# zihuixue/DynMM

Hardware: AMD Instinct MI355X
Metric: images/sec fwd+bwd, 480x640 RGB-D, batch 32/GPU (higher is better)
Workload: dtype f32; 1 GPU; configs[2]: zero-grad + fwd + weighted 4-scale CE + FLOP loss + bwd + fused SGD-Nesterov update, --dynamic --global-gate soft DiffSoftmax gates tau=1; per_gpu_batch=32, global_batch=32, height=480, width=640, parallelism=dp1, launch=eager, streams=4, optimizer_in_step=fused SGD-Nesterov

## Files before the change

### dynmm_amd/lib.py

```python
import ctypes as C
import os
import subprocess

_HERE = os.path.dirname(os.path.abspath(__file__))
LIB_PATH = os.path.join(_HERE, 'libdynmm_hip.so')
CSRC = os.path.join(_HERE, 'csrc')

ACT_NONE, ACT_RELU, ACT_TANH, ACT_SWISH, ACT_HSWISH = 0, 1, 2, 3, 4
SMOOTH_ACTS = (ACT_SWISH, ACT_HSWISH)
DYNMM_OK, DYNMM_EINVAL, DYNMM_EUNSUPPORTED, DYNMM_EWORKSPACE = 0, -1, -2, -3
ACT = {None: 0, 'none': 0, 'relu': 1, 'tanh': 2, 'swish': 3, 'silu': 3, 'hswish': 4}
LOSS_BCE_LOGITS, LOSS_L1 = 0, 1

c_f = C.c_void_p
c_i = C.c_int
c_fl = C.c_float
c_sz = C.c_size_t
c_ll = C.c_longlong


class ConvGeom(C.Structure):
    _fields_ = [(n, C.c_int) for n in ('N', 'Ci', 'H', 'W', 'Co', 'Ho', 'Wo',
                                       'KH', 'KW', 'SH', 'SW', 'PH', 'PW', 'c_split')]


class Dropout(C.Structure):
    _fields_ = [('mask', C.c_void_p), ('step', C.c_void_p), ('seed', C.c_ulonglong), ('offset', C.c_ulonglong),
                ('p', C.c_float)]


_GP = C.POINTER(ConvGeom)
_DP = C.POINTER(Dropout)
_PP = C.POINTER(C.c_void_p)
_IP = C.POINTER(C.c_int)

SIGNATURES = {
    'dynmm_abi_version': (c_i, []),
    'dynmm_build_info': (C.c_char_p, []),
    'dynmm_debug_set_igemm_v5': (c_i, [c_i]),
    'dynmm_conv2d_uses_operand_ring': (c_i, [_GP, c_i]),
    'dynmm_packed_weight_floats': (c_sz, [c_i, c_i, c_i, c_i, c_i]),
    'dynmm_pack_weight': (c_i, [c_f, c_f, c_f, c_i, c_i, c_i, c_i, c_f]),
    'dynmm_pack_weight_multi': (c_i, [c_f, c_f, c_f, c_i, c_i, c_f]),
    'dynmm_pack_weight_multi_blocks': (c_i, [c_i] * 5),
    'dynmm_conv2d_fwd': (c_i, [c_f, c_f, c_f, c_f, c_f, c_f, c_f, _GP, c_i, c_f]),
    'dynmm_conv2d_stem_fwd_stats_supported': (c_i, [_GP]),
    'dynmm_conv2d_stem_fwd_stats': (c_i, [c_f, c_f, c_f, c_f, c_f, _GP, c_f]),
    'dynmm_conv2d_dgrad': (c_i, [c_f, c_f, c_f, c_f, c_f, c_f, _GP, c_f]),
    'dynmm_conv2d_wino_supported': (c_i, [_GP, c_i]),
    'dynmm_wino_packed_floats': (c_sz, [c_i, c_i, c_i, c_i]),
    'dynmm_wino_pack': (c_i, [c_f, c_f, c_f, c_i, c_i, c_i, c_i, c_i, c_f]),
    'dynmm_wino_pack_multi_blocks': (c_i, [c_i] * 4),
    'dynmm_wino_pack_multi': (c_i, [c_f, c_f, c_f, c_i, c_i, c_f]),
    'dynmm_conv2d_wino_fwd': (c_i, [c_f, c_f, c_f, c_f, c_f, _GP, c_i, c_f]),
    'dynmm_conv2d_wino_dgrad_bnred_supported': (c_i, [_GP]),
    'dynmm_conv2d_wino_dgrad_bnred_slots': (c_i, [_GP]),
    'dynmm_conv2d_wino_dgrad_bnred': (c_i, [c_f] * 9 + [_GP, c_f]),
    'dynmm_conv2d_wino_dgrad_bnred2': (c_i, [c_f] * 9 + [_GP, c_f]),
    'dynmm_conv2d_wino_fwd_stats_supported': (c_i, [_GP]),
    'dynmm_conv2d_wino_fwd_stats_slots': (c_i, [_GP]),
    'dynmm_conv2d_wino_fwd_stats': (c_i, [c_f, c_f, c_f, c_f, c_f, c_i, _GP, c_f]),
    'dynmm_conv2d_wino_dgrad': (c_i, [c_f, c_f, c_f, c_f, c_f, _GP, c_f]),
    'dynmm_conv2d_wino2d_supported': (c_i, [_GP, c_i]),
    'dynmm_wino2d_packed_floats': (c_sz, [c_i, c_i]),
    'dynmm_wino2d_pack': (c_i, [c_f, c_f, c_f, c_i, c_i, c_i, c_f]),
    'dynmm_wino2d_pack_multi_blocks': (c_i, [c_i, c_i, c_i]),
    'dynmm_wino2d_pack_multi': (c_i, [c_f, c_f, c_f, c_i, c_i, c_f]),
    'dynmm_conv2d_wino2d_stats_slots': (c_i, [_GP]),
    'dynmm_conv2d_wino2d_fwd': (c_i, [c_f, c_f, c_f, c_f, c_f, c_f, c_i, _GP, c_i, c_f]),
    'dynmm_conv2d_wino2d_dgrad': (c_i, [c_f, c_f, c_f, c_f, c_f, _GP, c_f]),
    'dynmm_conv2d_wino43_supported': (c_i, [_GP]),
    'dynmm_wino43_packed_floats': (c_sz, [c_i, c_i, c_i, c_i]),
    'dynmm_wino43_pack': (c_i, [c_f, c_f, c_i, c_i, c_i, c_i, c_f]),
    'dynmm_wino43_pack_multi_blocks': (c_i, [c_i] * 4),
    'dynmm_wino43_pack_multi': (c_i, [c_f, c_f, c_f, c_i, c_i, c_f]),
    'dynmm_conv2d_wino43_dgrad': (c_i, [c_f, c_f, c_f, c_f, c_f, _GP, c_f]),
    'dynmm_conv2d_wgrad_workspace_bytes': (c_sz, [_GP]),
    'dynmm_conv2d_wgrad': (c_i, [c_f, c_f, c_f, c_f, c_f, c_f, c_sz, _GP, c_f]),
    'dynmm_conv2d_wgrad_groupable': (c_i, [_GP]),
    'dynmm_conv2d_wgrad_variant': (c_i, [_GP]),
    'dynmm_conv2d_wgrad_group_workspace_bytes': (c_sz, [_GP, c_i]),
    'dynmm_conv2d_wgrad_group': (c_i, [c_i, c_f, c_f, c_f, c_f, c_f, c_sz, _GP, c_f]),
    'dynmm_act_bwd_bias_workspace_bytes': (c_sz, [c_i, c_i]),
    'dynmm_act_bwd_bias': (c_i, [c_f, c_f, c_f, c_f, c_f, c_i, c_i, c_i, c_i, c_f]),
    'dynmm_act_pre_fwd': (c_i, [c_f, c_f, c_i, c_i, c_i, c_i, c_f]),
    'dynmm_act_pre_bwd': (c_i, [c_f, c_f, c_f, c_f, c_f, c_i, c_i, c_i, c_i, c_f]),
    'dynmm_bn_stats': (c_i, [c_f, c_f, c_i, c_i, c_i, c_i, c_f]),
    'dynmm_bn_stats_f64': (c_i, [c_f, c_f, c_i, c_i, c_i, c_i, c_f]),
    'dynmm_bn_relu_bits_words': (c_sz, [c_i, c_i, c_i]),
    'dynmm_bn_apply': (c_i, [c_f] * 11 + [c_i, c_i, c_i, c_fl, c_fl, c_i, c_i, c_f, c_f]),
    'dynmm_bn_bwd_reduce': (c_i, [c_f] * 8 + [c_i, c_i, c_i, c_i, c_i, c_f, c_f]),
    'dynmm_bn_bwd_apply': (c_i, [c_f] * 12 + [c_i, c_i, c_i, c_i, c_i, c_f, c_f]),
    'dynmm_bn_bwd_reduce_pre': (c_i, [c_f] * 8 + [c_i, c_i, c_i, c_i, c_i, c_f]),
    'dynmm_bn_bwd_apply_pre': (c_i, [c_f] * 12 + [c_i, c_i, c_i, c_i, c_i, c_f]),
    'dynmm_bn_fold': (c_i, [c_f] * 7 + [c_i, c_fl, c_f]),
    'dynmm_maxpool3x3s2_fwd': (c_i, [c_f, c_f, c_f] + [c_i] * 6 + [c_f]),
    'dynmm_maxpool3x3s2_bwd': (c_i, [c_f, c_f, c_f] + [c_i] * 6 + [c_f]),
    'dynmm_adaptive_avgpool_fwd': (c_i, [c_f, c_f] + [c_i] * 5 + [c_f]),
    'dynmm_adaptive_avgpool_bwd': (c_i, [c_f, c_f] + [c_i] * 5 + [c_f]),
    'dynmm_nearest_into_fwd': (c_i, [c_f, c_f] + [c_i] * 8 + [c_f]),
    'dynmm_nearest_into_bwd': (c_i, [c_f, c_f] + [c_i] * 8 + [c_f]),
# ... 176 lines not shown
```

### dynmm_amd/nn/blocks.py

```python
import torch
import torch.nn as nn

from .. import ops

ACTIVATIONS = {'relu': 'relu', 'swish': 'swish', 'silu': 'swish', 'hswish': 'hswish'}


def normalize_activation(activation):
    key = activation.lower() if isinstance(activation, str) else activation
    if key not in ACTIVATIONS:
        raise NotImplementedError('Only relu, swish and hswish as activation function are supported so far. '
                                  'Got {}'.format(activation))
    return ACTIVATIONS[key]


def conv_bn_act(x, conv, bn, act=None, residual=None, x2=None, mask_input=False, conv_link=None, res_link=None, bwd_link=None):
    if not bn.training and not torch.is_grad_enabled():
        return ops.conv2d_fused_eval(x, conv.weight, conv.bias, bn, act, residual,
                                     conv.stride, conv.padding, x2)
    y = ops.conv2d(x, conv.weight, conv.bias, conv.stride, conv.padding, None, x2, mask_input=mask_input, link=conv_link,
                   bn_stats=bn.training)
    return ops.batch_norm_act(y, bn, act, residual, link=res_link, bwd_link=bwd_link)


class ConvBNAct(nn.Sequential):

    def __init__(self, cin, cout, kernel_size, activation='relu'):
        super().__init__()
        self.activation = normalize_activation(activation)
        self.add_module('conv', nn.Conv2d(cin, cout, kernel_size, padding=kernel_size // 2, bias=False))
        self.add_module('bn', nn.BatchNorm2d(cout))

    def forward(self, x):
        return conv_bn_act(x, self.conv, self.bn, self.activation)


class NonBottleneck1D(nn.Module):
    expansion = 1

    def __init__(self, inplanes, planes, stride=1, downsample=None, activation='relu'):
        super().__init__()
        self.activation = normalize_activation(activation)
        self.conv3x1_1 = nn.Conv2d(inplanes, planes, (3, 1), stride=(stride, 1), padding=(1, 0))
        self.conv1x3_1 = nn.Conv2d(planes, planes, (1, 3), stride=(1, stride), padding=(0, 1))
        self.bn1 = nn.BatchNorm2d(planes, eps=1e-3)
        self.conv3x1_2 = nn.Conv2d(planes, planes, (3, 1), padding=(1, 0))
        self.conv1x3_2 = nn.Conv2d(planes, planes, (1, 3), padding=(0, 1))
        self.bn2 = nn.BatchNorm2d(planes, eps=1e-3)
        self.downsample = downsample

    def forward(self, x, chain=False):
        act = self.activation
        grad = torch.is_grad_enabled() and x.requires_grad
        fuse_bwd = grad and act == 'relu'
        link = ops.GradLink() if (grad and self.downsample is None) else None
        in_link = getattr(x, '_bn_out_link', None) if (chain and link is not None and fuse_bwd) else None
        xd = x
        if self.downsample is not None:
            x, xd = ops.fan_out(x, 2)
        c = self.conv3x1_1
        y = ops.conv2d(x, c.weight, c.bias, c.stride, c.padding, act, defer_mask=fuse_bwd, link=link, bn_link=in_link)
        bnl = ops.BNLink() if (fuse_bwd and self.bn1.training) else None
        y = conv_bn_act(y, self.conv1x3_1, self.bn1, act, mask_input=fuse_bwd, bwd_link=bnl)
        c = self.conv3x1_2
        y = ops.conv2d(y, c.weight, c.bias, c.stride, c.padding, act, defer_mask=fuse_bwd, bn_link=bnl)
        idt = x if self.downsample is None else conv_bn_act(xd, self.downsample[0], self.downsample[1])
        out_link = ops.BNLink() if (fuse_bwd and self.bn2.training) else None
        out = conv_bn_act(y, self.conv1x3_2, self.bn2, act, residual=idt, mask_input=fuse_bwd, res_link=link, bwd_link=out_link)
        if out_link is not None and out_link.bits is not None:
            out._bn_out_link = out_link
        return out


class BasicBlock(nn.Module):
    expansion = 1

    def __init__(self, inplanes, planes, stride=1, downsample=None, activation='relu'):
        super().__init__()
        self.activation = normalize_activation(activation)
        self.conv1 = nn.Conv2d(inplanes, planes, 3, stride=stride, padding=1, bias=False)
        self.bn1 = nn.BatchNorm2d(planes)
        self.conv2 = nn.Conv2d(planes, planes, 3, padding=1, bias=False)
        self.bn2 = nn.BatchNorm2d(planes)
        self.downsample = downsample

    def forward(self, x, chain=False):
        fuse_bwd = torch.is_grad_enabled() and x.requires_grad
        link = ops.GradLink() if (fuse_bwd and self.downsample is None) else None
        xd = x
        if self.downsample is not None:
            x, xd = ops.fan_out(x, 2)
        y = conv_bn_act(x, self.conv1, self.bn1, self.activation, conv_link=link)
        idt = x if self.downsample is None else conv_bn_act(xd, self.downsample[0], self.downsample[1])
        return conv_bn_act(y, self.conv2, self.bn2, self.activation, residual=idt, res_link=link)


class Bottleneck(nn.Module):
    expansion = 4

    def __init__(self, inplanes, planes, stride=1, downsample=None, activation='relu'):
        super().__init__()
        self.activation = normalize_activation(activation)
        self.conv1 = nn.Conv2d(inplanes, planes, 1, bias=False)
        self.bn1 = nn.BatchNorm2d(planes)
        self.conv2 = nn.Conv2d(planes, planes, 3, stride=stride, padding=1, bias=False)
        self.bn2 = nn.BatchNorm2d(planes)
        self.conv3 = nn.Conv2d(planes, planes * self.expansion, 1, bias=False)
        self.bn3 = nn.BatchNorm2d(planes * self.expansion)
        self.downsample = downsample

    def forward(self, x, chain=False):
        fuse_bwd = torch.is_grad_enabled() and x.requires_grad
        link = ops.GradLink() if (fuse_bwd and self.downsample is None) else None
        xd = x
        if self.downsample is not None:
            x, xd = ops.fan_out(x, 2)
        y = conv_bn_act(x, self.conv1, self.bn1, self.activation, conv_link=link)
        y = conv_bn_act(y, self.conv2, self.bn2, self.activation)
        idt = x if self.downsample is None else conv_bn_act(xd, self.downsample[0], self.downsample[1])
        return conv_bn_act(y, self.conv3, self.bn3, self.activation, residual=idt, res_link=link)


def chain_ok(prev, blk):
    import torch.nn.modules.module as M
    if prev._forward_hooks or blk._forward_pre_hooks:
        return False
    if M._global_forward_hooks or M._global_forward_pre_hooks:
        return False
    return True


BLOCKS = {'NonBottleneck1D': NonBottleneck1D, 'BasicBlock': BasicBlock, 'Bottleneck': Bottleneck}
LAYERS = {'resnet18': (2, 2, 2, 2), 'resnet34': (3, 4, 6, 3), 'resnet50': (3, 4, 6, 3)}


class ResNetEncoder(nn.Module):

    def __init__(self, name, block, input_channels=3, activation='relu'):
        super().__init__()
        self.activation = normalize_activation(activation)
        if name not in LAYERS:
            raise NotImplementedError(f'Only {sorted(LAYERS)} encoders are implemented on the HIP path. Got {name}')
        if block not in BLOCKS and name != 'resnet50':
            raise NotImplementedError(f'Block {block} is not implemented')
        if name == 'resnet50':
            block = 'Bottleneck'
        blk = BLOCKS[block]
        ex = blk.expansion
        self.conv1 = nn.Conv2d(input_channels, 64, 7, stride=2, padding=3, bias=False)
        self.bn1 = nn.BatchNorm2d(64)
        inplanes = 64
        for j, (planes, n) in enumerate(zip((64, 128, 256, 512), LAYERS[name]), start=1):
            stride = 1 if j == 1 else 2
            down = None
            if stride != 1 or inplanes != planes * ex:
                down = nn.Sequential(nn.Conv2d(inplanes, planes * ex, 1, stride=stride, bias=False),
                                     nn.BatchNorm2d(planes * ex))
            stage = [blk(inplanes, planes, stride, down, activation=self.activation)] + \
                [blk(planes * ex, planes, activation=self.activation) for _ in range(n - 1)]
            setattr(self, f'layer{j}', nn.Sequential(*stage))
            inplanes = planes * ex
        self.down_2_channels_out = 64
        self.down_4_channels_out, self.down_8_channels_out = 64 * ex, 128 * ex
        self.down_16_channels_out, self.down_32_channels_out = 256 * ex, 512 * ex
        for m in self.modules():
            if isinstance(m, nn.Conv2d):
                nn.init.kaiming_normal_(m.weight, mode='fan_out', nonlinearity='relu')
            elif isinstance(m, nn.BatchNorm2d):
                nn.init.constant_(m.weight, 1)
                nn.init.constant_(m.bias, 0)

    def forward_first_conv(self, x):
# ... 20 lines not shown
```

### dynmm_amd/ops.py

```python
import collections
import contextlib
import ctypes as C

import torch
from torch.autograd import Function

from . import lib as L

ACT = L.ACT


def _lib():
    return L.load()


def _stream():
    if not torch.cuda.is_available():
        raise L.DynmmHipError('no HIP device is available: the DynMM hot path runs only on its HIP kernels '
                              '(there is no CPU / eager-PyTorch fallback)')
    h = torch.cuda.current_stream().cuda_stream
    _CENSUS.add(h)
    return h


# ... 478 lines not shown

@contextlib.contextmanager
def capture_scope():
    import gc
    was = gc.isenabled()
    gc.collect()
    gc.disable()
    try:
        yield
    finally:
        if was:
            gc.enable()


ACT_TRACE = None

PROFILE = None


def _tile(co, m=1 << 30):
    if co > 64:
        return '128x32' if -(-co // 128) * -(-m // 64) < 3 * 256 else '128x64'
    return '64x128' if co > 32 else '32x256'




def _timed(kind, g, call, nprob=1, extra=0, route='direct'):
    if PROFILE is None:
        return call()
    co = g.Ci if kind == 'dgrad' else g.Co
    gemm_ci = g.Co if kind == 'dgrad' else g.Ci
    rk = ((gemm_ci + 15) & ~15) if (gemm_ci >= 8 and gemm_ci % 16) else gemm_ci
    generic = ''
    if kind != 'wgrad':
        if rk % 16 != 0 or (g.c_split < g.Ci and g.c_split % 16 != 0):
            generic = ',generic'
        elif rk != gemm_ci:
            generic = ',padded'
    m = g.N * (g.H * g.W if kind == 'dgrad' else g.Ho * g.Wo)
    name = f'conv_wgrad<co{_tile(co).split("x")[0]}>' if kind == 'wgrad' else f'conv_igemm_{kind}<{_tile(co, m)}{generic}>'
    if kind == 'wgrad':
        variant = _lib().dynmm_conv2d_wgrad_variant(C.byref(g))
        if variant == 6 and (g.SH == 2 or g.SW == 2):
            name = f'conv_wgrad_s2<co{128 if g.Co % 128 == 0 else 64},{g.KH}x{g.KW}>'
        elif variant == 6:
            name = f'conv_wgrad_v6<co{128 if g.Co % 128 == 0 else 64},{g.KH}x{g.KW}>'
        elif variant == 4:
            name = 'conv_wgrad_v4<co128>'
        elif variant == 8:
            name = 'conv_co8_wgrad<direct,valu>'
    if kind != 'wgrad' and not generic and _lib().dynmm_conv2d_uses_operand_ring(C.byref(g), int(kind == 'dgrad')):
        name = f'conv_igemm_v5_{kind}<{"128x64" if co % 128 == 0 else "64x128"},kw{g.KW}>'
    if route == 'wino2d':
        name = f'conv_wino2d_{kind}<co{128 if co % 128 == 0 else 64},3x3>'
    elif route != 'direct':
        name = f'conv_wino{"43" if route == "wino43" else ""}_{kind}<co{128 if co % 128 == 0 else 64},{g.KH}x{g.KW}{"s2" if g.SH * g.SW > 1 else ""}>'
    if kind == 'fwd':
        k5, k7 = (g.KH, g.KW, g.SH, g.SW, g.PH, g.PW) == (5, 5, 2, 2, 0, 0), (g.KH, g.KW, g.SH, g.SW, g.PH, g.PW) == (7, 7, 2, 2, 3, 3)
        if k5 and 5 <= g.Co <= 8 and g.Ci % 4 == 0 and g.Ci >= 16 and (g.c_split == g.Ci or g.c_split % (g.Ci // 4) == 0):
            name = 'conv_co8_fwd<direct,valu>'
        elif k7 and g.Ci in (1, 3) and g.Co == 64 and g.c_split == g.Ci:
            name = f'conv_stem_fwd<ci{g.Ci},mfma>'
    flops = 2.0 * g.N * g.Ho * g.Wo * g.KH * g.KW * g.Ci * g.Co * nprob
    e0, e1 = torch.cuda.Event(enable_timing=True), torch.cuda.Event(enable_timing=True)
    e0.record()
    r = call()
    e1.record()
    PROFILE.append((name, flops, e0, e1, (g.N, g.Ci, g.H, g.W, g.Co, g.KH, g.KW, g.SH, g.SW, nprob), (kind, int(extra))))
    return r


def _up4(v):
    return (v + 3) & ~3


def _pair(v):
    return (v, v) if isinstance(v, int) else tuple(v)


def _same_shape(a, b, what):
    if b is not None and tuple(a.shape) != tuple(b.shape):
        raise L.DynmmHipError(f'{what}: shape mismatch {tuple(a.shape)} vs {tuple(b.shape)}')


def _geom(x, x2, weight, stride, padding):
    if x.dim() != 4 or weight.dim() != 4:
        raise L.DynmmHipError('conv2d expects NCHW input and OIHW weight')
    if x2 is not None and (x2.shape[0] != x.shape[0] or tuple(x2.shape[2:]) != tuple(x.shape[2:])):
        raise L.DynmmHipError(f'conv2d: second input {tuple(x2.shape)} does not match {tuple(x.shape)}')
    N, C0, H, W = x.shape
    Ci = C0 + (x2.shape[1] if x2 is not None else 0)
    Co, Ciw, KH, KW = weight.shape
    if Ciw != Ci:
        raise L.DynmmHipError(f'conv2d: weight expects {Ciw} input channels, got {Ci}')
    SH, SW = stride
    PH, PW = padding
    Ho = (H + 2 * PH - KH) // SH + 1
    Wo = (W + 2 * PW - KW) // SW + 1
    if N <= 0 or Ho <= 0 or Wo <= 0:
        raise L.DynmmHipError(f'conv2d: empty output for input {tuple(x.shape)}, kernel {(KH, KW)}, stride {stride}, '
                              f'padding {padding}')
    g = L.ConvGeom(N, Ci, H, W, Co, Ho, Wo, KH, KW, SH, SW, PH, PW, C0)
    return g


class GradLink:
    __slots__ = ('dres',)

    def __init__(self):
        self.dres = None


class BNLink:
    __slots__ = ('x', 'mean', 'invstd', 'gamma', 'beta', 'sums', 'bits', 'premasked')

    def __init__(self):
        self.x = self.mean = self.invstd = self.gamma = self.beta = self.sums = self.bits = None
        self.premasked = False


BN_BWD_FUSE = True
BN_RELU_BITS = True


_PackedEntry = collections.namedtuple('_PackedEntry', 'weight Co Ci KH KW kinds')


class PackedWeights:

    def __init__(self):
        self.reg = {}
        self.slots = {}
        self.arena = None
        self.launches = []
        self.valid = False
        self.dirty = False

    def register(self, weight, g, kinds):
        if not isinstance(weight, torch.nn.Parameter):
            return
        e = self.reg.get(id(weight))
        if e is None:
            e = self.reg[id(weight)] = _PackedEntry(weight, g.Co, g.Ci, g.KH, g.KW, set())
        if not e.kinds.issuperset(kinds):
            e.kinds.update(kinds)
            self.dirty = True

    def lookup(self, weight, kinds):
        ops = self.slots.get(id(weight)) if self.valid else None
        if ops is not None:
            for kind in kinds:
                if kind not in ops:
                    return None
        return ops

    def _layout(self):
        lib = _lib()
        ents = list(self.reg.values())
        dev = ents[0].weight.device
        base = min(e.weight.data_ptr() for e in ents)
        off = 0
        rows = {name: [] for name in ('pack_weight',) + tuple(f.name + '_pack' for f in _PACK_FAMILIES)}
        blk = dict.fromkeys(rows, 0)
# ... 42 lines not shown


def _planes(t):
    if t.dim() >= 2:
        return t.shape[0], t.shape[1], max(t.numel() // max(t.shape[0] * t.shape[1], 1), 1)
    return 1, max(t.numel(), 1), 1


class _Activation(Function):

    @staticmethod
    def forward(ctx, z, act):
        z = _chk(z, 'z')
        a = torch.empty_like(z)
        if z.numel():
            N, Cc, HW = _planes(z)
            L.check(_lib().dynmm_act_pre_fwd(_p(z), _p(a), N, Cc, HW, act, _stream()), 'act_pre_fwd')
        ctx.act = act
        ctx.save_for_backward(z)
        return a

    @staticmethod
    def backward(ctx, g):
        z, = ctx.saved_tensors
        g = _chk(g, 'grad')
        dz = torch.empty_like(z)
        if z.numel():
            N, Cc, HW = _planes(z)
            L.check(_lib().dynmm_act_pre_bwd(_p(g), _p(z), _p(dz), None, None, N, Cc, HW, ctx.act, _stream()), 'act_pre_bwd')
        return dz, None


def is_smooth(act):
    return ACT[act] in L.SMOOTH_ACTS


def activation(x, act):
    code = ACT[act]
    if code == L.ACT_NONE:
        return x
    if not (torch.is_grad_enabled() and x.requires_grad):
        x = _chk(x, 'x')
        a = torch.empty_like(x)
        if x.numel():
            N, Cc, HW = _planes(x)
            L.check(_lib().dynmm_act_pre_fwd(_p(x), _p(a), N, Cc, HW, code, _stream()), 'act_pre_fwd')
        return a
    return _Activation.apply(x, code)


class _Conv2d(Function):
    @staticmethod
    def forward(ctx, x, x2, weight, bias, stride, padding, act, mask_input, defer_mask, link, w_owner=None, stats=None,
                bn_link=None):
        lib = _lib()
        st = _stream()
        x, x2, weight, bias = _chk(x, 'x'), _chk(x2, 'x2'), _chk(weight, 'weight'), _chk(bias, 'bias')
        g = _geom(x, x2, weight, stride, padding)
        need_dx = ctx.needs_input_grad[0] or (x2 is not None and ctx.needs_input_grad[1])
        y = torch.empty((g.N, g.Co, g.Ho, g.Wo), device=x.device, dtype=torch.float32)
        fwd = _fwd_route(g, x2, x.data_ptr() % 16 == 0)
        dgrad = _dgrad_route(g, x2) if need_dx else None
        kinds = (_FWD_KIND[fwd], _DGRAD_KIND[dgrad]) if need_dx else (_FWD_KIND[fwd],)
        wkey = w_owner if w_owner is not None else weight
        prepack = _STEP.prepack if _STEP is not None else None
        packed = prepack.lookup(wkey, kinds) if prepack is not None else None
        if packed is None:
            packed = _pack_operands(weight, g, kinds)
            if prepack is not None:
                prepack.register(wkey, g, kinds)
        wf = packed[kinds[0]]
        if fwd == 'wino2d':
            sums, ns = None, 0
            if stats is not None and act == L.ACT_NONE and g.Co % 64 == 0:
                ns = lib.dynmm_conv2d_wino2d_stats_slots(C.byref(g))
                stats['sums'] = sums = _zeroed_sums(2 * g.Co * ns, x.device)
            L.check(_timed('fwd', g, lambda: lib.dynmm_conv2d_wino2d_fwd(_p(x), _p(wf), _p(bias), None, _p(y), _p(sums), ns,
                                                                         C.byref(g), act, st), route=fwd), 'conv2d_wino2d_fwd')
        elif (fwd == 'wino' and stats is not None and act == L.ACT_NONE and g.KW == 3 and
                lib.dynmm_conv2d_wino_fwd_stats_supported(C.byref(g))):
            ns = lib.dynmm_conv2d_wino_fwd_stats_slots(C.byref(g))
            sums = _zeroed_sums(2 * g.Co * ns, x.device)
            L.check(_timed('fwd', g, lambda: lib.dynmm_conv2d_wino_fwd_stats(_p(x), _p(wf), _p(bias), _p(y), _p(sums), ns,
                                                                             C.byref(g), st), route=fwd), 'conv2d_wino_fwd_stats')
            stats['sums'] = sums
        elif fwd == 'wino':
            L.check(_timed('fwd', g, lambda: lib.dynmm_conv2d_wino_fwd(_p(x), _p(wf), _p(bias), None, _p(y), C.byref(g), act, st),
                           route=fwd), 'conv2d_wino_fwd')
        elif (stats is not None and act == L.ACT_NONE and x2 is None and
                lib.dynmm_conv2d_stem_fwd_stats_supported(C.byref(g))):
            sums = _zeroed_sums(2 * g.Co, x.device)
            L.check(_timed('fwd', g, lambda: lib.dynmm_conv2d_stem_fwd_stats(_p(x), _p(wf), _p(bias), _p(y), _p(sums),
                                                                             C.byref(g), st)), 'conv2d_stem_fwd_stats')
            stats['sums'] = sums
        else:
            L.check(_timed('fwd', g, lambda: lib.dynmm_conv2d_fwd(_p(x), _p(x2), _p(wf), None, _p(bias), None, _p(y),
                                                                  C.byref(g), act, st)), 'conv2d_fwd')
        ctx.geom = g
        ctx.act = act
        ctx.has_bias = bias is not None
        ctx.has_x2 = x2 is not None
        ctx.dgrad_route = dgrad
        ctx.mask_input = mask_input
        ctx.defer_mask = defer_mask
        ctx.link = link
        ctx.bn_link = bn_link
        ctx.save_for_backward(x, x2, packed[kinds[1]] if need_dx else None, y if (act != L.ACT_NONE and not defer_mask) else None)
        ctx.wshape = tuple(weight.shape)
        ctx.w_param, ctx.b_param = (w_owner if w_owner is not None else weight), bias
        return y

    @staticmethod
    def backward(ctx, gy):
        lib = _lib()
        st = _stream()
        x, x2, wpd, y = ctx.saved_tensors
        g = ctx.geom
        gy = _chk(gy, 'grad')
        dbias = None
        act = L.ACT_NONE if ctx.defer_mask else ctx.act
        dbias_ret = None
        bias_in_wgrad = ctx.has_bias and ctx.needs_input_grad[2]
        defer = (ctx.needs_input_grad[2] and x2 is None and
                 _wgrad_grouped(g, ctx.w_param, *([ctx.b_param] if ctx.has_bias else [])))
        if ctx.has_bias and not (defer and bias_in_wgrad):
            dbias, dbias_ret = _grad_dst(ctx.b_param)
        if act != L.ACT_NONE or (ctx.has_bias and not bias_in_wgrad):
            ge = torch.empty_like(gy) if act != L.ACT_NONE else None
            wsb = None
            if not bias_in_wgrad and dbias is not None:
                nb = lib.dynmm_act_bwd_bias_workspace_bytes(g.N, g.Co)
                wsb = torch.empty(max(nb // 4, 1), device=gy.device, dtype=torch.float32)
            L.check(lib.dynmm_act_bwd_bias(_p(gy), _p(y), _p(ge), None if bias_in_wgrad else _p(dbias), _p(wsb),
                                           g.N, g.Co, g.Ho * g.Wo, act, st), 'act_bwd_bias')
            if ge is not None:
                gy = ge
        dx = dx2 = None
        if wpd is not None:
            dx = torch.empty_like(x)
            dx2 = torch.empty_like(x2) if x2 is not None else None
            mask = x if ctx.mask_input else None
            accum = None
            if ctx.link is not None and ctx.link.dres is not None:
                accum, ctx.link.dres = ctx.link.dres, None
            extra = (mask is not None) + (accum is not None)
            route = ctx.dgrad_route
            if route != 'direct':
                gyw = gy if gy.data_ptr() % 16 == 0 else gy.clone()
                mask, accum = (t if (t is None or t.data_ptr() % 16 == 0) else t.clone() for t in (mask, accum))
                bl = ctx.bn_link
                if (bl is not None and bl.x is not None and bl.bits is not None and route in _WINO_F23 and mask is None and
                        (ctx.link is None) == (accum is None) and
                        bl.x.data_ptr() % 8 == 0 and (g.H * g.W) % 4 == 0 and
                        lib.dynmm_conv2d_wino_dgrad_bnred_supported(C.byref(g))):
                    sums = _zeroed_sums(2 * g.Ci * lib.dynmm_conv2d_wino_dgrad_bnred_slots(C.byref(g)), dx.device)
                    L.check(_timed('dgrad', g, lambda: lib.dynmm_conv2d_wino_dgrad_bnred2(
                        _p(gyw), _p(wpd), _p(accum), _p(bl.x), _p(bl.bits), _p(bl.mean), _p(bl.invstd), _p(sums), _p(dx),
                        C.byref(g), st), extra=2, route=route), 'conv2d_wino_dgrad_bnred2')
                    bl.sums, bl.premasked = sums, True
                elif (bl is not None and bl.x is not None and bl.bits is None and route in _WINO_F23 and mask is None and
                        accum is None and
                        bl.x.data_ptr() % 8 == 0 and lib.dynmm_conv2d_wino_dgrad_bnred_supported(C.byref(g))):
                    sums = _zeroed_sums(2 * g.Ci * lib.dynmm_conv2d_wino_dgrad_bnred_slots(C.byref(g)), dx.device)
                    L.check(_timed('dgrad', g, lambda: lib.dynmm_conv2d_wino_dgrad_bnred(
                        _p(gyw), _p(wpd), _p(bl.x), _p(bl.mean), _p(bl.invstd), _p(bl.gamma), _p(bl.beta), _p(sums), _p(dx),
                        C.byref(g), st), extra=1, route=route), 'conv2d_wino_dgrad_bnred')
                    bl.sums = sums
                else:
                    fn = {'wino2d': lib.dynmm_conv2d_wino2d_dgrad, 'wino43': lib.dynmm_conv2d_wino43_dgrad}.get(route, lib.dynmm_conv2d_wino_dgrad)
                    L.check(_timed('dgrad', g, lambda: fn(_p(gyw), _p(wpd), _p(mask), _p(accum), _p(dx), C.byref(g), st),
                                   extra=extra, route=route), 'conv2d_wino_dgrad')
            else:
                L.check(_timed('dgrad', g, lambda: lib.dynmm_conv2d_dgrad(_p(gy), _p(wpd), _p(mask), _p(accum), _p(dx),
                                                                          _p(dx2), C.byref(g), st), extra=extra), 'conv2d_dgrad')
        dw_ret = None
        ws_stream = None
        _age_wgrad_queues()
        if defer:
            _queue_wgrad(g, x, gy, ctx.w_param, ctx.b_param if bias_in_wgrad else None)
        elif ctx.needs_input_grad[2]:
            dw, dw_ret = _grad_dst(ctx.w_param)
            nbytes = lib.dynmm_conv2d_wgrad_workspace_bytes(C.byref(g))
            if dw_ret is None and _STEP.async_wgrad and PROFILE is None:
                ws_stream = _wgrad_stream()
                _CENSUS.add(ws_stream.cuda_stream)
                ws_stream.wait_stream(torch.cuda.current_stream())
                with torch.cuda.stream(ws_stream):
                    ws = torch.empty(max(nbytes // 4, 1), device=gy.device, dtype=torch.float32)
                    L.check(lib.dynmm_conv2d_wgrad(_p(x), _p(x2), _p(gy), _p(dw), _p(dbias) if bias_in_wgrad else None,
                                                   _p(ws), nbytes, C.byref(g), ws_stream.cuda_stream), 'conv2d_wgrad')
                _STEP.inflight.append((x, x2, gy))
            else:
                ws = torch.empty(max(nbytes // 4, 1), device=gy.device, dtype=torch.float32)
                L.check(_timed('wgrad', g, lambda: lib.dynmm_conv2d_wgrad(_p(x), _p(x2), _p(gy), _p(dw),
                                                                          _p(dbias) if bias_in_wgrad else None, _p(ws), nbytes,
                                                                          C.byref(g), st)), 'conv2d_wgrad')
        _grads_enqueued(torch.cuda.current_stream(), ws_stream)
        if dw_ret is not None and tuple(dw_ret.shape) != ctx.wshape:
            dw_ret = dw_ret.reshape(ctx.wshape)
        return dx, dx2, dw_ret, dbias_ret, None, None, None, None, None, None, None, None, None


def conv2d(x, weight, bias=None, stride=1, padding=0, act=None, x2=None, mask_input=False, defer_mask=False,
           link=None, w_owner=None, bn_stats=False, bn_link=None):
    if is_smooth(act) and (torch.is_grad_enabled() or not isinstance(weight, torch.nn.Parameter) or w_owner is not None):
        z = conv2d(x, weight, bias, stride, padding, None, x2, link=link, w_owner=w_owner)
        return activation(z, act)
    if not torch.is_grad_enabled() and isinstance(weight, torch.nn.Parameter) and w_owner is None:
        return conv2d_fused_eval(x, weight, bias, None, act, None, stride, padding, x2)
    holder = {} if (bn_stats and CONV_BN_STATS and x2 is None) else None
    y = _Conv2d.apply(x, x2, weight, bias, _pair(stride), _pair(padding), ACT[act], bool(mask_input),
                      bool(defer_mask), link, w_owner, holder, bn_link if BN_BWD_FUSE else None)
    if holder:
        y._bn_sums = holder['sums']
    if ACT_TRACE is not None and ACT[act] == L.ACT_RELU:
        ACT_TRACE.append(y.detach())
    return y


class _FanOut(Function):

    @staticmethod
    def forward(ctx, x, n):
        return tuple(x.view_as(x) for _ in range(n))

    @staticmethod
    def backward(ctx, *gs):
        gs = [_chk(g, 'grad') for g in gs if g is not None]
        if not gs:
            return None, None
        if len(gs) == 1:
            return gs[0], None
        out = torch.empty_like(gs[0])
        while len(gs) > 1:
            take, gs = gs[:4], gs[4:]
            dst = out if not gs else torch.empty_like(out)
            L.check(_lib().dynmm_add_n(_ptr_array(take), len(take), _p(dst), C.c_size_t(dst.numel()), _stream()), 'add_n')
            gs = [dst] + gs
        return out, None


_NO_FANOUT = False


def fan_out(x, n):
    if n <= 1 or _NO_FANOUT or not (torch.is_grad_enabled() and x.requires_grad):
        return (x,) * n
    return _FanOut.apply(x, n)


_MUTATION_GEN = [0]


def note_mutation():
    _MUTATION_GEN[0] += 1


CAPTURE_EVAL_CACHE = False
_EVAL_CACHE = {'direct': '_dynmm_eval_cache', 'wino': '_dynmm_eval_cache_wino', 'wino2d': '_dynmm_eval_cache_wino2d'}


def conv2d_fused_eval(x, weight, conv_bias, bn, act=None, residual=None, stride=1, padding=0, x2=None):
    lib = _lib()
    st = _stream()
    x, x2, weight = _chk(x, 'x'), _chk(x2, 'x2'), _chk(weight, 'weight')
# ... 1319 lines not shown
```

### include/dynmm_hip.h

```cpp
#ifndef DYNMM_HIP_H
#define DYNMM_HIP_H

#include <stddef.h>

#ifdef __cplusplus
extern "C" {
#endif

#define DYNMM_OK 0
#define DYNMM_EINVAL (-1)
#define DYNMM_EUNSUPPORTED (-2)
#define DYNMM_EWORKSPACE (-3)

#define DYNMM_ACT_NONE 0
#define DYNMM_ACT_RELU 1
#define DYNMM_ACT_TANH 2
#define DYNMM_ACT_SWISH 3
#define DYNMM_ACT_HSWISH 4

#define DYNMM_LOSS_BCE_LOGITS 0
#define DYNMM_LOSS_L1 1

int dynmm_abi_version(void);
const char* dynmm_build_info(void);

int dynmm_debug_set_igemm_v5(int mode);

typedef struct {
    int N, Ci, H, W;
    int Co, Ho, Wo;
    int KH, KW, SH, SW, PH, PW;
    int c_split;
} dynmm_conv_geom;

int dynmm_conv2d_uses_operand_ring(const dynmm_conv_geom* g, int dgrad);

size_t dynmm_packed_weight_floats(int Co, int Ci, int KH, int KW, int dgrad);
int dynmm_pack_weight(const float* w, float* wp_fwd, float* wp_dgrad,
                      int Co, int Ci, int KH, int KW, void* stream);

int dynmm_pack_weight_multi_blocks(int Co, int Ci, int KH, int KW, int dgrad);
int dynmm_pack_weight_multi(const float* src_base, float* dst_base, const void* desc, int ndesc, int total_blocks,
                            void* stream);

int dynmm_conv2d_fwd(const float* x, const float* x2, const float* wp_fwd,
                     const float* scale, const float* shift, const float* residual,
                     float* y, const dynmm_conv_geom* g, int act, void* stream);

int dynmm_conv2d_stem_fwd_stats_supported(const dynmm_conv_geom* g);
int dynmm_conv2d_stem_fwd_stats(const float* x, const float* wp_fwd, const float* bias, float* y, double* stats,
                                const dynmm_conv_geom* g, void* stream);

int dynmm_conv2d_dgrad(const float* dy, const float* wp_dgrad, const float* mask, const float* accum,
                       float* dx, float* dx2, const dynmm_conv_geom* g, void* stream);

int dynmm_conv2d_wino_supported(const dynmm_conv_geom* g, int dgrad);
size_t dynmm_wino_packed_floats(int Co, int Ci, int KH, int KW);
int dynmm_wino_pack(const float* w, float* ut, const float* scale ,
                    int Co, int Ci, int KH, int KW, int dgrad, void* stream);
int dynmm_wino_pack_multi_blocks(int Co, int Ci, int KH, int KW);
int dynmm_wino_pack_multi(const float* src_base, float* dst_base, const void* desc, int ndesc, int total_blocks,
                          void* stream);
int dynmm_conv2d_wino_fwd(const float* x, const float* ut, const float* bias, const float* residual, float* y,
                          const dynmm_conv_geom* g, int act, void* stream);
int dynmm_conv2d_wino_dgrad_bnred_supported(const dynmm_conv_geom* g);
int dynmm_conv2d_wino_dgrad_bnred_slots(const dynmm_conv_geom* g);
int dynmm_conv2d_wino_dgrad_bnred(const float* dy, const float* ut, const float* bn_x, const float* bn_mean,
                                  const float* bn_invstd, const float* bn_gamma, const float* bn_beta, double* sums, float* dx,
                                  const dynmm_conv_geom* g, void* stream);
int dynmm_conv2d_wino_dgrad_bnred2(const float* dy, const float* ut, const float* accum, const float* bn_x,
                                   const unsigned long long* relu_bits, const float* bn_mean, const float* bn_invstd,
                                   double* sums, float* dx, const dynmm_conv_geom* g, void* stream);
int dynmm_conv2d_wino_fwd_stats_supported(const dynmm_conv_geom* g);
int dynmm_conv2d_wino_fwd_stats_slots(const dynmm_conv_geom* g);
int dynmm_conv2d_wino_fwd_stats(const float* x, const float* ut, const float* bias, float* y, double* stats, int nslots,
                                const dynmm_conv_geom* g, void* stream);
int dynmm_conv2d_wino_dgrad(const float* dy, const float* ut, const float* mask, const float* accum, float* dx,
                            const dynmm_conv_geom* g, void* stream);

int dynmm_conv2d_wino2d_supported(const dynmm_conv_geom* g, int dgrad);
size_t dynmm_wino2d_packed_floats(int Co, int Ci);
int dynmm_wino2d_pack(const float* w, float* ut, const float* scale, int Co, int Ci, int dgrad, void* stream);
int dynmm_wino2d_pack_multi_blocks(int Co, int Ci, int dgrad);
int dynmm_wino2d_pack_multi(const float* src_base, float* dst_base, const void* desc, int ndesc, int total_blocks, void* stream);
int dynmm_conv2d_wino2d_stats_slots(const dynmm_conv_geom* g);
int dynmm_conv2d_wino2d_fwd(const float* x, const float* ut, const float* bias, const float* residual, float* y, double* stats,
                            int nslots, const dynmm_conv_geom* g, int act, void* stream);
int dynmm_conv2d_wino2d_dgrad(const float* dy, const float* ut, const float* mask, const float* accum, float* dx,
                              const dynmm_conv_geom* g, void* stream);

int dynmm_conv2d_wino43_supported(const dynmm_conv_geom* g);
size_t dynmm_wino43_packed_floats(int Co, int Ci, int KH, int KW);
int dynmm_wino43_pack(const float* w, float* ut, int Co, int Ci, int KH, int KW, void* stream);
int dynmm_wino43_pack_multi_blocks(int Co, int Ci, int KH, int KW);
int dynmm_wino43_pack_multi(const float* src_base, float* dst_base, const void* desc, int ndesc, int total_blocks,
                            void* stream);
int dynmm_conv2d_wino43_dgrad(const float* dy, const float* ut, const float* mask, const float* accum, float* dx,
                              const dynmm_conv_geom* g, void* stream);

size_t dynmm_conv2d_wgrad_workspace_bytes(const dynmm_conv_geom* g);
int dynmm_conv2d_wgrad(const float* x, const float* x2, const float* dy, float* dw, float* dbias,
                       void* workspace, size_t workspace_bytes,
                       const dynmm_conv_geom* g, void* stream);

int dynmm_conv2d_wgrad_groupable(const dynmm_conv_geom* g);
int dynmm_conv2d_wgrad_variant(const dynmm_conv_geom* g);
size_t dynmm_conv2d_wgrad_group_workspace_bytes(const dynmm_conv_geom* g, int n);
// ... 331 lines not shown
```

Before: 526.5 images/s.

## Accumulate 1x1 stride-2 shortcut dgrad directly into main-branch input gradient

Adds an MFMA kernel that computes the 1x1 stride-2 downsample conv's input gradient and adds it in place into the dx buffer already produced by the main-branch conv dgrad. A ShortcutLink coordinates the two backward calls, whichever runs first, so the shortcut branch no longer allocates its own dx, the fan_out gradient sum is skipped, and the strided scatter is fused into the accumulate. This removes an allocation, a separate dgrad launch and an elementwise add per downsampling block. In exchange it adds cross-Function state, a stream wait when the two branches ran on different streams, and fallback paths that must stay correct.

```diff
diff --git a/dynmm_amd/csrc/conv_shortcut.hip b/dynmm_amd/csrc/conv_shortcut.hip
--- /dev/null
+++ b/dynmm_amd/csrc/conv_shortcut.hip
@@ -0,0 +1,176 @@
+#include "common.h"
+#include "mfma.h"
+
+namespace dynmm {
+
+namespace {
+
+struct ShortcutArgs {
+    const float* dy;
+    const float* w;
+    float* dx;
+    int Ci, Co, H, W, Ho, Wo;
+    int M;
+    int n_ci_tiles;
+};
+
+template <int NT, bool VEC>
+__global__ void __launch_bounds__(256, NT == 128 ? 5 : 1) conv1x1_s2_dgrad_acc_kernel(const ShortcutArgs a) {
+    constexpr int MT = 64, BK = 16;
+    constexpr int NB = NT / 64;
+    constexpr int QR = NT / 4;
+    constexpr int BQ = BK * QR / 256;
+    constexpr int KS = 256 / QR;
+    __shared__ __attribute__((aligned(16))) float As[2][BK * MT];
+    __shared__ __attribute__((aligned(16))) float Bs[2][BK * NT];
+
+    const int t = threadIdx.x;
+    const int lane = t & 63;
+    const int wave = __builtin_amdgcn_readfirstlane(t >> 6);
+    const int wm = wave & 1, wn = wave >> 1;
+    const int l31 = lane & 31, khalf = lane >> 5;
+
+    const int lin = xcd_remap(blockIdx.x, gridDim.x);
+    const int ci0 = (lin % a.n_ci_tiles) * MT;
+    const int m0 = (lin / a.n_ci_tiles) * NT;
+    const int HWo = a.Ho * a.Wo;
+
+    const int ka = t >> 4, ca = ci0 + 4 * (t & 15);
+    const int kb = t / QR, qb = t % QR;
+    size_t boff[VEC ? 1 : 4];
+    bool bin[VEC ? 1 : 4];
+#pragma unroll
+    for (int e = 0; e < (VEC ? 1 : 4); ++e) {
+        const int m = m0 + 4 * qb + e;
+        bin[e] = m < a.M;
+        const int n = bin[e] ? m / HWo : 0;
+        boff[e] = (size_t)n * a.Co * HWo + (size_t)(bin[e] ? m - n * HWo : 0);
+    }
+
+    float4 ra, rb[BQ];
+    auto load = [&](int k0) __attribute__((always_inline)) {
+        const int co = k0 + ka;
+        ra = make_float4(0.f, 0.f, 0.f, 0.f);
+        if (co < a.Co) {
+            const float* p = a.w + (size_t)co * a.Ci + ca;
+            if constexpr (VEC) {
+                if (ca < a.Ci) ra = *reinterpret_cast<const float4*>(p);
+            } else {
+                if (ca < a.Ci) ra.x = p[0];
+                if (ca + 1 < a.Ci) ra.y = p[1];
+                if (ca + 2 < a.Ci) ra.z = p[2];
+                if (ca + 3 < a.Ci) ra.w = p[3];
+            }
+        }
+#pragma unroll
+        for (int i = 0; i < BQ; ++i) {
+            const int cb = k0 + kb + KS * i;
+            rb[i] = make_float4(0.f, 0.f, 0.f, 0.f);
+            if (cb < a.Co) {
+                const float* p = a.dy + (size_t)cb * HWo;
+                if constexpr (VEC) {
+                    if (bin[0]) rb[i] = *reinterpret_cast<const float4*>(p + boff[0]);
+                } else {
+                    if (bin[0]) rb[i].x = p[boff[0]];
+                    if (bin[1]) rb[i].y = p[boff[1]];
+                    if (bin[2]) rb[i].z = p[boff[2]];
+                    if (bin[3]) rb[i].w = p[boff[3]];
+                }
+            }
+        }
+    };
+    auto stage = [&](int buf) __attribute__((always_inline)) {
+        *reinterpret_cast<float4*>(&As[buf][ka * MT + 4 * (t & 15)]) = ra;
+#pragma unroll
+        for (int i = 0; i < BQ; ++i) *reinterpret_cast<float4*>(&Bs[buf][(kb + KS * i) * NT + 4 * qb]) = rb[i];
+    };
+
+    f32x16 acc[NB];
+#pragma unroll
+    for (int b = 0; b < NB; ++b)
+#pragma unroll
+        for (int r = 0; r < 16; ++r) acc[b][r] = 0.f;
+
+    const int nsteps = (a.Co + BK - 1) / BK;
+    load(0);
+    stage(0);
+    __syncthreads();
+    for (int s = 0; s < nsteps; ++s) {
+        const int buf = s & 1;
+        if (s + 1 < nsteps) load((s + 1) * BK);
+        const float* As_ = &As[buf][32 * wm + l31];
+        const float* Bs_ = &Bs[buf][(NT / 2) * wn + l31];
+#pragma unroll
+        for (int k2 = 0; k2 < BK / 2; ++k2) {
+            const int k = 2 * k2 + khalf;
+            const float av = As_[k * MT];
+#pragma unroll
+            for (int b = 0; b < NB; ++b) acc[b] = mfma_32x32x2(av, Bs_[k * NT + 32 * b], acc[b]);
+        }
+        if (s + 1 < nsteps) stage(buf ^ 1);
+        __syncthreads();
+    }
+
+    const size_t HW = (size_t)a.H * a.W;
+#pragma unroll
+    for (int b = 0; b < NB; ++b) {
+        const int m = m0 + (NT / 2) * wn + 32 * b + l31;
+        if (m >= a.M) continue;
+        const int n = m / HWo, p = m - n * HWo;
+        const int ho = p / a.Wo, wo = p - ho * a.Wo;
+        float* d = a.dx + (size_t)n * a.Ci * HW + (size_t)(2 * ho) * a.W + 2 * wo;
+        const int cbase = ci0 + 32 * wm + 4 * khalf;
+        float v[16];
+#pragma unroll
+        for (int r = 0; r < 16; ++r) {
+            const int ci = cbase + 8 * (r >> 2) + (r & 3);
+            v[r] = ci < a.Ci ? d[(size_t)ci * HW] : 0.f;
+        }
+#pragma unroll
+        for (int r = 0; r < 16; ++r) {
+            const int ci = cbase + 8 * (r >> 2) + (r & 3);
+            if (ci < a.Ci) d[(size_t)ci * HW] = v[r] + acc[b][r];
+        }
+    }
+}
+
+bool shortcut_shape_ok(const dynmm_conv_geom* g) {
+    if (g->N <= 0 || g->Ci <= 0 || g->Co <= 0 || g->H <= 0 || g->W <= 0) return false;
+    if (g->KH != 1 || g->KW != 1 || g->SH != 2 || g->SW != 2 || g->PH != 0 || g->PW != 0 || g->c_split != g->Ci) return false;
+    if (g->Ho != (g->H - 1) / 2 + 1 || g->Wo != (g->W - 1) / 2 + 1) return false;
+    const unsigned long long m = (unsigned long long)g->N * g->Ho * g->Wo;
+    if (m >= (1ull << 31) - 128) return false;
+    if ((m + 63) / 64 * (unsigned long long)((g->Ci + 63) / 64) >= (1ull << 31)) return false;
+    return true;
+}
+
+}
+
+}
+
+using namespace dynmm;
+
+extern "C" int dynmm_conv1x1_s2_dgrad_acc_supported(const dynmm_conv_geom* g) { return g && shortcut_shape_ok(g) ? 1 : 0; }
+
+extern "C" int dynmm_conv1x1_s2_dgrad_acc(const float* dy, const float* w, float* dx, const dynmm_conv_geom* g, void* stream) {
+    if (!dy || !w || !dx || !g) return DYNMM_EINVAL;
+    if (!shortcut_shape_ok(g)) return DYNMM_EUNSUPPORTED;
+    hipStream_t st = (hipStream_t)stream;
+    ShortcutArgs a;
+    a.dy = dy; a.w = w; a.dx = dx;
+    a.Ci = g->Ci; a.Co = g->Co; a.H = g->H; a.W = g->W; a.Ho = g->Ho; a.Wo = g->Wo;
+    a.M = g->N * g->Ho * g->Wo;
+    a.n_ci_tiles = ceil_div(g->Ci, 64);
+    const bool vec = g->Ci % 4 == 0 && (g->Ho * g->Wo) % 4 == 0 && (uintptr_t)dy % 16 == 0 && (uintptr_t)w % 16 == 0;
+    const bool wide = (long long)a.n_ci_tiles * ceil_div(a.M, 128) >= 1024;
+    const dim3 grid((unsigned)(a.n_ci_tiles * ceil_div(a.M, wide ? 128 : 64)));
+    if (wide) {
+        if (vec) hipLaunchKernelGGL((conv1x1_s2_dgrad_acc_kernel<128, true>), grid, dim3(256), 0, st, a);
+        else hipLaunchKernelGGL((conv1x1_s2_dgrad_acc_kernel<128, false>), grid, dim3(256), 0, st, a);
+    } else {
+        if (vec) hipLaunchKernelGGL((conv1x1_s2_dgrad_acc_kernel<64, true>), grid, dim3(256), 0, st, a);
+        else hipLaunchKernelGGL((conv1x1_s2_dgrad_acc_kernel<64, false>), grid, dim3(256), 0, st, a);
+    }
+    DYNMM_LAUNCH_CHECK();
+    return DYNMM_OK;
+}
diff --git a/dynmm_amd/lib.py b/dynmm_amd/lib.py
--- a/dynmm_amd/lib.py
+++ b/dynmm_amd/lib.py
@@ -47,6 +47,8 @@
     'dynmm_conv2d_stem_fwd_stats_supported': (c_i, [_GP]),
     'dynmm_conv2d_stem_fwd_stats': (c_i, [c_f, c_f, c_f, c_f, c_f, _GP, c_f]),
     'dynmm_conv2d_dgrad': (c_i, [c_f, c_f, c_f, c_f, c_f, c_f, _GP, c_f]),
+    'dynmm_conv1x1_s2_dgrad_acc_supported': (c_i, [_GP]),
+    'dynmm_conv1x1_s2_dgrad_acc': (c_i, [c_f, c_f, c_f, _GP, c_f]),
     'dynmm_conv2d_wino_supported': (c_i, [_GP, c_i]),
     'dynmm_wino_packed_floats': (c_sz, [c_i, c_i, c_i, c_i]),
     'dynmm_wino_pack': (c_i, [c_f, c_f, c_f, c_i, c_i, c_i, c_i, c_i, c_f]),
diff --git a/dynmm_amd/nn/blocks.py b/dynmm_amd/nn/blocks.py
--- a/dynmm_amd/nn/blocks.py
+++ b/dynmm_amd/nn/blocks.py
@@ -14,13 +14,24 @@
     return ACTIVATIONS[key]
 
 
-def conv_bn_act(x, conv, bn, act=None, residual=None, x2=None, mask_input=False, conv_link=None, res_link=None, bwd_link=None):
+def conv_bn_act(x, conv, bn, act=None, residual=None, x2=None, mask_input=False, conv_link=None, res_link=None, bwd_link=None,
+                shortcut_link=None):
     if not bn.training and not torch.is_grad_enabled():
         return ops.conv2d_fused_eval(x, conv.weight, conv.bias, bn, act, residual,
                                      conv.stride, conv.padding, x2)
     y = ops.conv2d(x, conv.weight, conv.bias, conv.stride, conv.padding, None, x2, mask_input=mask_input, link=conv_link,
-                   bn_stats=bn.training)
+                   bn_stats=bn.training, shortcut_link=shortcut_link)
     return ops.batch_norm_act(y, bn, act, residual, link=res_link, bwd_link=bwd_link)
+
+
+def block_input(x, downsample, grad):
+    if downsample is None:
+        return x, x, None
+    c = downsample[0]
+    if grad and ops.SHORTCUT_ACC and (c.kernel_size, c.stride, c.padding) == ((1, 1), (2, 2), (0, 0)):
+        x = x.view_as(x)
+        return x, x, ops.ShortcutLink()
+    return (*ops.fan_out(x, 2), None)
 
 
 class ConvBNAct(nn.Sequential):
@@ -55,16 +66,15 @@
         fuse_bwd = grad and act == 'relu'
         link = ops.GradLink() if (grad and self.downsample is None) else None
         in_link = getattr(x, '_bn_out_link', None) if (chain and link is not None and fuse_bwd) else None
-        xd = x
-        if self.downsample is not None:
-            x, xd = ops.fan_out(x, 2)
+        x, xd, sl = block_input(x, self.downsample, grad)
         c = self.conv3x1_1
-        y = ops.conv2d(x, c.weight, c.bias, c.stride, c.padding, act, defer_mask=fuse_bwd, link=link, bn_link=in_link)
+        y = ops.conv2d(x, c.weight, c.bias, c.stride, c.padding, act, defer_mask=fuse_bwd, link=link, bn_link=in_link,
+                       shortcut_link=sl)
         bnl = ops.BNLink() if (fuse_bwd and self.bn1.training) else None
         y = conv_bn_act(y, self.conv1x3_1, self.bn1, act, mask_input=fuse_bwd, bwd_link=bnl)
         c = self.conv3x1_2
         y = ops.conv2d(y, c.weight, c.bias, c.stride, c.padding, act, defer_mask=fuse_bwd, bn_link=bnl)
-        idt = x if self.downsample is None else conv_bn_act(xd, self.downsample[0], self.downsample[1])
+        idt = x if self.downsample is None else conv_bn_act(xd, self.downsample[0], self.downsample[1], shortcut_link=sl)
         out_link = ops.BNLink() if (fuse_bwd and self.bn2.training) else None
         out = conv_bn_act(y, self.conv1x3_2, self.bn2, act, residual=idt, mask_input=fuse_bwd, res_link=link, bwd_link=out_link)
         if out_link is not None and out_link.bits is not None:
@@ -87,11 +97,9 @@
     def forward(self, x, chain=False):
         fuse_bwd = torch.is_grad_enabled() and x.requires_grad
         link = ops.GradLink() if (fuse_bwd and self.downsample is None) else None
-        xd = x
-        if self.downsample is not None:
-            x, xd = ops.fan_out(x, 2)
-        y = conv_bn_act(x, self.conv1, self.bn1, self.activation, conv_link=link)
-        idt = x if self.downsample is None else conv_bn_act(xd, self.downsample[0], self.downsample[1])
+        x, xd, sl = block_input(x, self.downsample, fuse_bwd)
+        y = conv_bn_act(x, self.conv1, self.bn1, self.activation, conv_link=link, shortcut_link=sl)
+        idt = x if self.downsample is None else conv_bn_act(xd, self.downsample[0], self.downsample[1], shortcut_link=sl)
         return conv_bn_act(y, self.conv2, self.bn2, self.activation, residual=idt, res_link=link)
 
 
@@ -112,12 +120,10 @@
     def forward(self, x, chain=False):
         fuse_bwd = torch.is_grad_enabled() and x.requires_grad
         link = ops.GradLink() if (fuse_bwd and self.downsample is None) else None
-        xd = x
-        if self.downsample is not None:
-            x, xd = ops.fan_out(x, 2)
-        y = conv_bn_act(x, self.conv1, self.bn1, self.activation, conv_link=link)
+        x, xd, sl = block_input(x, self.downsample, fuse_bwd)
+        y = conv_bn_act(x, self.conv1, self.bn1, self.activation, conv_link=link, shortcut_link=sl)
         y = conv_bn_act(y, self.conv2, self.bn2, self.activation)
-        idt = x if self.downsample is None else conv_bn_act(xd, self.downsample[0], self.downsample[1])
+        idt = x if self.downsample is None else conv_bn_act(xd, self.downsample[0], self.downsample[1], shortcut_link=sl)
         return conv_bn_act(y, self.conv3, self.bn3, self.activation, residual=idt, res_link=link)
 
 
diff --git a/dynmm_amd/ops.py b/dynmm_amd/ops.py
--- a/dynmm_amd/ops.py
+++ b/dynmm_amd/ops.py
@@ -554,7 +554,9 @@
             name = 'conv_co8_wgrad<direct,valu>'
     if kind != 'wgrad' and not generic and _lib().dynmm_conv2d_uses_operand_ring(C.byref(g), int(kind == 'dgrad')):
         name = f'conv_igemm_v5_{kind}<{"128x64" if co % 128 == 0 else "64x128"},kw{g.KW}>'
-    if route == 'wino2d':
+    if route == 's2acc':
+        name = f'conv1x1_s2_dgrad_acc<64x{128 if -(-g.Ci // 64) * -(-g.N * g.Ho * g.Wo // 128) >= 1024 else 64}>'
+    elif route == 'wino2d':
         name = f'conv_wino2d_{kind}<co{128 if co % 128 == 0 else 64},3x3>'
     elif route != 'direct':
         name = f'conv_wino{"43" if route == "wino43" else ""}_{kind}<co{128 if co % 128 == 0 else 64},{g.KH}x{g.KW}{"s2" if g.SH * g.SW > 1 else ""}>'
@@ -612,6 +614,47 @@
 
     def __init__(self):
         self.dres = None
+
+
+SHORTCUT_ACC = True
+
+
+class ShortcutLink:
+    __slots__ = ('key', 'has_main', 'has_shortcut', 'broken', 'pending', 'dx', 'main_done')
+
+    def __init__(self):
+        self.key = None
+        self.has_main = self.has_shortcut = self.broken = self.main_done = False
+        self.pending = self.dx = None
+
+    def enlist(self, x, shortcut):
+        key = (x.data_ptr(), tuple(x.shape), tuple(x.stride()))
+        if self.key is None:
+            self.key = key
+        taken = self.has_shortcut if shortcut else self.has_main
+        if self.broken or taken or key != self.key:
+            self.broken = True
+            return None
+        if shortcut:
+            self.has_shortcut = True
+        else:
+            self.has_main = True
+        return 'shortcut' if shortcut else 'main'
+
+    @property
+    def armed(self):
+        return self.has_main and self.has_shortcut and not self.broken
+
+
+def _shortcut_acc(gy, weight, dx, g):
+    lib = _lib()
+    st = _stream()
+    L.check(_timed('dgrad', g, lambda: lib.dynmm_conv1x1_s2_dgrad_acc(_p(gy), _p(weight), _p(dx), C.byref(g), st), route='s2acc'),
+            'conv1x1_s2_dgrad_acc')
+
+
+def _acc_target_ok(dx):
+    return dx.dtype == torch.float32 and dx.is_contiguous() and dx.data_ptr() % 4 == 0
 
 
 class BNLink:
@@ -760,7 +803,7 @@
 class _Conv2d(Function):
     @staticmethod
     def forward(ctx, x, x2, weight, bias, stride, padding, act, mask_input, defer_mask, link, w_owner=None, stats=None,
-                bn_link=None):
+                bn_link=None, shortcut_link=None):
         lib = _lib()
         st = _stream()
         x, x2, weight, bias = _chk(x, 'x'), _chk(x2, 'x2'), _chk(weight, 'weight'), _chk(bias, 'bias')
@@ -813,6 +856,15 @@
         ctx.defer_mask = defer_mask
         ctx.link = link
         ctx.bn_link = bn_link
+        ctx.sc_link, ctx.sc_role, ctx.sc_weight = shortcut_link, None, None
+        if shortcut_link is not None:
+            shortcut = bool(lib.dynmm_conv1x1_s2_dgrad_acc_supported(C.byref(g)))
+            if (ctx.needs_input_grad[0] and x2 is None and not mask_input and
+                    ((w_owner is None and link is None) if shortcut else bn_link is None)):
+                ctx.sc_role = shortcut_link.enlist(x, shortcut)
+                ctx.sc_weight = weight if ctx.sc_role == 'shortcut' else None
+            else:
+                shortcut_link.broken = True
         ctx.save_for_backward(x, x2, packed[kinds[1]] if need_dx else None, y if (act != L.ACT_NONE and not defer_mask) else None)
         ctx.wshape = tuple(weight.shape)
         ctx.w_param, ctx.b_param = (w_owner if w_owner is not None else weight), bias
@@ -844,7 +896,18 @@
             if ge is not None:
                 gy = ge
         dx = dx2 = None
-        if wpd is not None:
+        sl = ctx.sc_link if ctx.sc_role is not None and ctx.sc_link.armed else None
+        absorbed = False
+        if sl is not None and ctx.sc_role == 'shortcut' and wpd is not None:
+            if sl.dx is not None:
+                (dxm, stream_m), sl.dx = sl.dx, None
+                if stream_m == st and _acc_target_ok(dxm):
+                    _shortcut_acc(gy, ctx.sc_weight, dxm, g)
+                    absorbed = True
+            elif not sl.main_done:
+                sl.pending = (gy, ctx.sc_weight, g, torch.cuda.current_stream())
+                absorbed = True
+        if wpd is not None and not absorbed:
             dx = torch.empty_like(x)
             dx2 = torch.empty_like(x2) if x2 is not None else None
             mask = x if ctx.mask_input else None
@@ -881,6 +944,15 @@
             else:
                 L.check(_timed('dgrad', g, lambda: lib.dynmm_conv2d_dgrad(_p(gy), _p(wpd), _p(mask), _p(accum), _p(dx),
                                                                           _p(dx2), C.byref(g), st), extra=extra), 'conv2d_dgrad')
+            if sl is not None and ctx.sc_role == 'main':
+                if sl.pending is not None:
+                    (gys, ws, gs, stream_s), sl.pending = sl.pending, None
+                    if stream_s.cuda_stream != st:
+                        torch.cuda.current_stream().wait_stream(stream_s)
+                    _shortcut_acc(gys, ws, dx, gs)
+                elif not sl.main_done and _acc_target_ok(dx):
+                    sl.dx = (dx, st)
+                sl.main_done = True
         dw_ret = None
         ws_stream = None
         _age_wgrad_queues()
@@ -906,19 +978,20 @@
         _grads_enqueued(torch.cuda.current_stream(), ws_stream)
         if dw_ret is not None and tuple(dw_ret.shape) != ctx.wshape:
             dw_ret = dw_ret.reshape(ctx.wshape)
-        return dx, dx2, dw_ret, dbias_ret, None, None, None, None, None, None, None, None, None
+        return dx, dx2, dw_ret, dbias_ret, None, None, None, None, None, None, None, None, None, None
 
 
 def conv2d(x, weight, bias=None, stride=1, padding=0, act=None, x2=None, mask_input=False, defer_mask=False,
-           link=None, w_owner=None, bn_stats=False, bn_link=None):
+           link=None, w_owner=None, bn_stats=False, bn_link=None, shortcut_link=None):
     if is_smooth(act) and (torch.is_grad_enabled() or not isinstance(weight, torch.nn.Parameter) or w_owner is not None):
-        z = conv2d(x, weight, bias, stride, padding, None, x2, link=link, w_owner=w_owner)
+        z = conv2d(x, weight, bias, stride, padding, None, x2, link=link, w_owner=w_owner, shortcut_link=shortcut_link)
         return activation(z, act)
     if not torch.is_grad_enabled() and isinstance(weight, torch.nn.Parameter) and w_owner is None:
         return conv2d_fused_eval(x, weight, bias, None, act, None, stride, padding, x2)
     holder = {} if (bn_stats and CONV_BN_STATS and x2 is None) else None
     y = _Conv2d.apply(x, x2, weight, bias, _pair(stride), _pair(padding), ACT[act], bool(mask_input),
-                      bool(defer_mask), link, w_owner, holder, bn_link if BN_BWD_FUSE else None)
+                      bool(defer_mask), link, w_owner, holder, bn_link if BN_BWD_FUSE else None,
+                      shortcut_link if SHORTCUT_ACC else None)
     if holder:
         y._bn_sums = holder['sums']
     if ACT_TRACE is not None and ACT[act] == L.ACT_RELU:
diff --git a/include/dynmm_hip.h b/include/dynmm_hip.h
--- a/include/dynmm_hip.h
+++ b/include/dynmm_hip.h
@@ -53,6 +53,9 @@
 
 int dynmm_conv2d_dgrad(const float* dy, const float* wp_dgrad, const float* mask, const float* accum,
                        float* dx, float* dx2, const dynmm_conv_geom* g, void* stream);
+
+int dynmm_conv1x1_s2_dgrad_acc_supported(const dynmm_conv_geom* g);
+int dynmm_conv1x1_s2_dgrad_acc(const float* dy, const float* w, float* dx, const dynmm_conv_geom* g, void* stream);
 
 int dynmm_conv2d_wino_supported(const dynmm_conv_geom* g, int dgrad);
 size_t dynmm_wino_packed_floats(int Co, int Ci, int KH, int KW);
```

Measured after the change: 528.2 images/s (median of 6 runs). Within noise of the previous version (+0.3%).
